# tudocomp/tudocomp

Measured on AMD Instinct MI355X. Metric: input MB/s end-to-end lcpcomp+huffman, higher is better.
Workload: dtype u32

## Files before the change

include/tdc_gpu.h:

```cpp
#ifndef TDC_GPU_H
#define TDC_GPU_H

#include <stddef.h>
#include <stdint.h>

#ifdef __cplusplus
extern "C" {
#endif

typedef enum {
    TDC_GPU_OK = 0,
    TDC_GPU_ERR_HIP = -1,
    TDC_GPU_ERR_ARG = -2,
    TDC_GPU_ERR_NO_SENTINEL = -3,
    TDC_GPU_ERR_TOO_LARGE = -4,
    TDC_GPU_ERR_OOM = -5,
    TDC_GPU_ERR_UNSUPPORTED = -6,
    TDC_GPU_ERR_INTERNAL = -7
} tdc_gpu_status;

enum { TDC_GPU_CODER_HUFF = 0, TDC_GPU_CODER_GAMMA = 1, TDC_GPU_CODER_ARITH = 2, TDC_GPU_CODER_ASCII = 3, TDC_GPU_CODER_SLE = 4,
       TDC_GPU_CODER_BIT = 5 , TDC_GPU_CODER_DELTA = 6  };
#define TDC_GPU_CODER_SLE_K(K) (TDC_GPU_CODER_SLE | ((K) << 8))
enum { TDC_GPU_COMP_ARRAYS = 0, TDC_GPU_COMP_PLCPPEAKS = 1, TDC_GPU_COMP_MAXLCP = 2, TDC_GPU_COMP_HEAP = 3 };
// ... 105 lines not shown
                                     size_t* out_len, uint64_t* factors, uint32_t* rounds);
int tdc_gpu_lzss_lcp_factorize(tdc_gpu_ctx* ctx, const uint8_t* text, size_t n, uint32_t threshold,
                               uint32_t** pos, uint32_t** src, uint32_t** len, size_t* z);

int tdc_gpu_sort_pairs_u64(tdc_gpu_ctx* ctx, uint64_t* keys, uint32_t* vals, size_t n, int algo);
int tdc_gpu_suffix_array(tdc_gpu_ctx* ctx, const uint8_t* text, size_t n, uint32_t* sa, uint32_t* isa);
int tdc_gpu_textds(tdc_gpu_ctx* ctx, const uint8_t* text, size_t n, uint32_t* sa, uint32_t* isa, uint32_t* phi,
                   uint32_t* plcp, uint32_t* lcp, uint32_t* maxlcp);
int tdc_gpu_lcpcomp_factorize(tdc_gpu_ctx* ctx, const uint8_t* text, size_t n, uint32_t threshold, int flatten,
                              uint32_t** pos, uint32_t** src, uint32_t** len, size_t* z, tdc_gpu_stats* stats);
int tdc_gpu_flatten(tdc_gpu_ctx* ctx, size_t n, const uint32_t* pos, uint32_t* src, const uint32_t* len, size_t z,
                    uint64_t* num_flattened, uint64_t* max_depth_lb);
int tdc_gpu_prim_scan(tdc_gpu_ctx* ctx, int op, void* data, size_t n, int in_place, void* total);
int tdc_gpu_prim_sort_pairs(tdc_gpu_ctx* ctx, int kind, void* keys, uint32_t* vals, size_t n, int begin_bit, int end_bit);
int tdc_gpu_prim_bucketed_scatter(tdc_gpu_ctx* ctx, const uint32_t* idx, const uint32_t* val, size_t m, uint32_t* dst, size_t n_dst,
                                  uint32_t fill, int permutation, int second_tmp, int offset);
int tdc_gpu_prim_msd_partition(tdc_gpu_ctx* ctx, uint32_t* idx, uint32_t* val, size_t m, int bits, int db);
int tdc_gpu_prim_select(tdc_gpu_ctx* ctx, const uint8_t* cls, uint8_t want, size_t m, const uint32_t* srcA, const uint64_t* srcB,
                        uint32_t fillA, uint64_t fillB, uint32_t* outA, uint64_t* outB, uint32_t* count);
int tdc_gpu_prim_select_counts(tdc_gpu_ctx* ctx, const uint8_t* cls, uint8_t want, size_t m, const uint32_t* srcA, const uint32_t* tile_counts,
                               uint32_t fillA, uint32_t* outA, uint32_t* count);
int tdc_gpu_prim_mark_orbit(tdc_gpu_ctx* ctx, const uint32_t* next, size_t n, uint8_t* mark);
int tdc_gpu_prim_tile_entries(tdc_gpu_ctx* ctx, const uint16_t* exit0, size_t ntiles, uint32_t states, uint16_t* entry0);
int tdc_gpu_prim_arena_fill(tdc_gpu_ctx* ctx, int byte, uint64_t* base, uint64_t* size);

int tdc_gpu_lcpcomp_decompress(tdc_gpu_ctx* ctx, const uint8_t* stream, size_t len, uint8_t** out, size_t* out_len,
                               uint64_t* factors, uint32_t* rounds);
int tdc_gpu_lcpcomp_decompress_coder(tdc_gpu_ctx* ctx, const uint8_t* stream, size_t len, int coder, uint8_t** out, size_t* out_len,
                                     uint64_t* factors, uint32_t* rounds);
int tdc_gpu_lcpcomp_decompress_into(tdc_gpu_ctx* ctx, const uint8_t* stream, size_t len, int coder, uint8_t* out, size_t out_cap,
                                    size_t* out_len, uint64_t* factors, uint32_t* rounds);
int tdc_gpu_ctx_last_decode_on_device(const tdc_gpu_ctx* ctx);

int tdc_gpu_lz78_decompress(tdc_gpu_ctx* ctx, const uint8_t* stream, size_t len, int coder, uint8_t** out, size_t* out_len,
                            uint64_t* phrases, uint32_t* rounds);
int tdc_gpu_lz78_decompress_into(tdc_gpu_ctx* ctx, const uint8_t* stream, size_t len, int coder, uint8_t* out, size_t out_cap,
                                 size_t* out_len, uint64_t* phrases, uint32_t* rounds);

int tdc_gpu_lzw_compress(tdc_gpu_ctx* ctx, const uint8_t* in, size_t n, int coder, uint8_t** out, size_t* out_len,
                         tdc_gpu_stats* stats);
int tdc_gpu_lzw_decompress(tdc_gpu_ctx* ctx, const uint8_t* stream, size_t len, int coder, uint8_t** out, size_t* out_len,
                           uint64_t* codes, uint32_t* rounds);
int tdc_gpu_lzw_decompress_into(tdc_gpu_ctx* ctx, const uint8_t* stream, size_t len, int coder, uint8_t* out, size_t out_cap,
                                size_t* out_len, uint64_t* codes, uint32_t* rounds);

int tdc_gpu_lzss_sw_compress(tdc_gpu_ctx* ctx, const uint8_t* in, size_t n, uint32_t window, uint32_t threshold, int coder,
// ... 113 lines not shown
```

tudocomp_amd/__init__.py:

```python
import ctypes

import numpy as np

from . import _native
from ._native import Stats, Stage, LIB_PATH, SYMBOLS

CODER_HUFF = 0
CODER_GAMMA = 1
CODER_ARITH = 2
CODER_ASCII = 3
CODER_SLE = 4
CODER_BIT = 5
CODER_DELTA = 6
COMP_ARRAYS = 0
COMP_PLCPPEAKS = 1
COMP_MAXLCP = 2
COMP_HEAP = 3
STAGE_BWT = 0
STAGE_RLE = 1
STAGE_MTF = 2
STAGE_HUFF = 3
STAGE_SLE = 4


# ... 791 lines not shown
            raise ValueError("one count per tile of 2048 classes")
        a = None if src_a is None else np.ascontiguousarray(src_a, dtype=np.uint32)
        if a is not None and len(a) != m:
            raise ValueError("cls and src_a differ in length")
        oa = np.empty(m, dtype=np.uint32)
        cnt = ctypes.c_uint32(0)
        self._check(self._L.tdc_gpu_prim_select_counts(self._h, _ptr(c), int(want), m, None if a is None else _ptr(a), _ptr(t),
                                                       int(fill_a), _ptr(oa), ctypes.byref(cnt)))
        return oa, cnt.value

    def prim_mark_orbit(self, nxt):
        a = np.ascontiguousarray(nxt, dtype=np.uint32)
        mark = np.empty(len(a), dtype=np.uint8)
        self._check(self._L.tdc_gpu_prim_mark_orbit(self._h, _ptr(a), len(a), _ptr(mark)))
        return mark

    def prim_tile_entries(self, exits):
        a = np.ascontiguousarray(exits, dtype=np.uint16)
        ntiles, states = a.shape
        entry = np.empty(ntiles, dtype=np.uint16)
        self._check(self._L.tdc_gpu_prim_tile_entries(self._h, _ptr(a), ntiles, states, _ptr(entry)))
        return entry

    def prim_arena_fill(self, byte=None):
        base, size = ctypes.c_uint64(), ctypes.c_uint64()
        self._check(self._L.tdc_gpu_prim_arena_fill(self._h, -1 if byte is None else int(byte), ctypes.byref(base), ctypes.byref(size)))
        return base.value, size.value

    def suffix_array(self, text):
        a = _u8(text)
        sa = np.empty(len(a), dtype=np.uint32)
        isa = np.empty(len(a), dtype=np.uint32)
        self._check(self._L.tdc_gpu_suffix_array(self._h, _ptr(a), len(a), _ptr(sa), _ptr(isa)))
        return sa, isa

    def textds(self, text):
        a = _u8(text)
        n = len(a)
        arrs = {k: np.empty(n, dtype=np.uint32) for k in ("sa", "isa", "phi", "plcp", "lcp")}
        m = ctypes.c_uint32()
        self._check(self._L.tdc_gpu_textds(self._h, _ptr(a), n, _ptr(arrs["sa"]), _ptr(arrs["isa"]), _ptr(arrs["phi"]),
                                           _ptr(arrs["plcp"]), _ptr(arrs["lcp"]), ctypes.byref(m)))
        arrs["maxlcp"] = m.value
        return arrs

    def lcpcomp_decompress(self, stream, coder=CODER_HUFF):
# ... 464 lines not shown
```

tudocomp_amd/_native.py:

```python
import ctypes
import os

_HERE = os.path.dirname(os.path.abspath(__file__))
LIB_PATH = os.environ.get("TDC_GPU_LIB") or os.path.join(_HERE, "lib", "libtdc_gpu.so")

SYMBOLS = [
    "tdc_gpu_ctx_create", "tdc_gpu_ctx_destroy", "tdc_gpu_ctx_reserve", "tdc_gpu_strerror", "tdc_gpu_last_error",
    "tdc_gpu_ctx_set_profiling", "tdc_gpu_ctx_reset_profile", "tdc_gpu_ctx_kernel_profile",
    "tdc_gpu_free", "tdc_gpu_lcpcomp_compress", "tdc_gpu_lcpcomp_compress_raw", "tdc_gpu_lcpcomp_compress_dev",
    "tdc_gpu_lcpcomp_bound", "tdc_gpu_lcpcomp_bound_coder", "tdc_gpu_lcpcomp_compress_into", "tdc_gpu_host_alloc", "tdc_gpu_host_free",
    "tdc_gpu_lz78_compress", "tdc_gpu_lzss_lcp_compress", "tdc_gpu_lzss_lcp_factorize",
    "tdc_gpu_sort_pairs_u64", "tdc_gpu_suffix_array", "tdc_gpu_textds", "tdc_gpu_lcpcomp_factorize", "tdc_gpu_flatten", "tdc_gpu_encode_huff",
    "tdc_gpu_prim_scan", "tdc_gpu_prim_sort_pairs", "tdc_gpu_prim_bucketed_scatter", "tdc_gpu_prim_msd_partition", "tdc_gpu_prim_select", "tdc_gpu_prim_select_counts",
    "tdc_gpu_prim_mark_orbit", "tdc_gpu_prim_tile_entries", "tdc_gpu_prim_arena_fill",
    "tdc_gpu_lcpcomp_decompress",
    "tdc_gpu_lcpcomp_compress_comp",
    "tdc_gpu_encode_arith",
    "tdc_gpu_encode_ascii",
    "tdc_gpu_encode_sle",
    "tdc_gpu_lcpcomp_decompress_coder", "tdc_gpu_ctx_last_decode_on_device", "tdc_gpu_lcpcomp_decompress_into",
    "tdc_gpu_ctx_set_option", "tdc_gpu_option_count", "tdc_gpu_option_name", "tdc_escape", "tdc_unescape", "tdc_lz78_factors", "tdc_huffman_table", "tdc_huffman_selfcheck", "tdc_gpu_blocks_count", "tdc_gpu_blocks_compress", "tdc_gpu_blocks_decompress", "tdc_gpu_device_count", "tdc_gen_english", "tdc_gen_dna",
    "tdc_gpu_arena_bytes", "tdc_gpu_device_memory",
    "tdc_gpu_lcpcomp_compress_keep", "tdc_gpu_stream_fetch", "tdc_gpu_stream_fetch_dev", "tdc_gpu_host_register", "tdc_gpu_host_unregister",
    "tdc_gpu_lz78_decompress", "tdc_gpu_lz78_decompress_into",
    "tdc_gpu_bwt_compress", "tdc_gpu_bwt_compress_into", "tdc_gpu_bwt_decompress", "tdc_gpu_bwt_decompress_into", "tdc_gpu_bwt_inverse_stage",
    "tdc_gpu_pipeline_bound", "tdc_gpu_pipeline_compress", "tdc_gpu_pipeline_compress_into", "tdc_gpu_pipeline_decompress",
    "tdc_gpu_pipeline_decompress_into", "tdc_gpu_pipeline_decompress_stats", "tdc_rle_decode", "tdc_mtf_decode", "tdc_huff_decode_literals", "tdc_sle_decode",
    "tdc_gpu_lzw_compress", "tdc_gpu_lzw_decompress", "tdc_gpu_lzw_decompress_into", "tdc_lzw_factors", "tdc_lzw_decode",
    "tdc_gpu_lzss_lcp_compress_into", "tdc_gpu_lzss_lcp_bound", "tdc_gpu_lzss_lcp_decompress", "tdc_gpu_lzss_lcp_decompress_into", "tdc_lzss_decode",
    "tdc_gpu_lzss_sw_compress", "tdc_gpu_lzss_sw_compress_into", "tdc_gpu_lzss_sw_bound", "tdc_gpu_lzss_sw_factorize", "tdc_lzss_sw_factors",
    "tdc_lzss_sw_decode", "tdc_gpu_lzss_sw_decompress", "tdc_gpu_lzss_sw_decompress_into",
    "tdc_gpu_lzss_sw_compress_batch", "tdc_gpu_lzss_sw_batch_bound", "tdc_gpu_lzss_sw_decompress_batch",
    "tdc_gpu_lzw_compress_batch", "tdc_gpu_lzw_batch_bound", "tdc_gpu_lz78_compress_batch", "tdc_gpu_lz78_batch_bound", "tdc_gpu_lz_parse_batch",
    "tdc_gpu_lzw_decompress_batch", "tdc_gpu_lz78_decompress_batch",
    "tdc_gpu_repair_compress", "tdc_gpu_repair_compress_into", "tdc_gpu_repair_bound", "tdc_gpu_repair_grammar", "tdc_gpu_repair_decompress",
    "tdc_gpu_repair_decompress_into", "tdc_gpu_repair_decompress_stats", "tdc_repair_grammar", "tdc_repair_decode",
]
# ... 81 lines not shown
    L.tdc_gpu_stream_fetch.argtypes = [vp, vp, sz, psz]
    L.tdc_gpu_stream_fetch_dev.argtypes = [vp, vp, sz, psz]
    L.tdc_gpu_ctx_last_decode_on_device.argtypes = [vp]
    L.tdc_gpu_lcpcomp_decompress_into.argtypes = [vp, vp, sz, i32, vp, sz, psz, ctypes.POINTER(ctypes.c_uint64), ctypes.POINTER(ctypes.c_uint32)]
    L.tdc_gpu_host_register.argtypes = [vp, sz]
    L.tdc_gpu_host_unregister.argtypes = [vp]
    L.tdc_gpu_blocks_count.argtypes = [sz, sz]
    L.tdc_gpu_blocks_count.restype = sz
    L.tdc_gpu_blocks_compress.argtypes = [ctypes.POINTER(i32), i32, vp, sz, sz, u32, i32, i32, pvp, psz, ctypes.POINTER(Stats)]
    L.tdc_gpu_blocks_decompress.argtypes = [vp, vp, sz, i32, pvp, psz]
    L.tdc_gpu_host_alloc.argtypes = [sz]
    L.tdc_gpu_host_alloc.restype = vp
    L.tdc_gpu_host_free.argtypes = [vp]
    L.tdc_gpu_host_free.restype = None
    L.tdc_gpu_sort_pairs_u64.argtypes = [vp, vp, vp, sz, i32]
    L.tdc_gpu_prim_scan.argtypes = [vp, i32, vp, sz, i32, vp]
    L.tdc_gpu_prim_sort_pairs.argtypes = [vp, i32, vp, vp, sz, i32, i32]
    L.tdc_gpu_prim_bucketed_scatter.argtypes = [vp, vp, vp, sz, vp, sz, u32, i32, i32, i32]
    L.tdc_gpu_prim_msd_partition.argtypes = [vp, vp, vp, sz, i32, i32]
    L.tdc_gpu_prim_select.argtypes = [vp, vp, ctypes.c_uint8, sz, vp, vp, u32, ctypes.c_uint64, vp, vp, ctypes.POINTER(u32)]
    L.tdc_gpu_prim_select_counts.argtypes = [vp, vp, ctypes.c_uint8, sz, vp, vp, u32, vp, ctypes.POINTER(u32)]
    L.tdc_gpu_prim_mark_orbit.argtypes = [vp, vp, sz, vp]
    L.tdc_gpu_prim_tile_entries.argtypes = [vp, vp, sz, u32, vp]
    L.tdc_gpu_prim_arena_fill.argtypes = [vp, i32, ctypes.POINTER(ctypes.c_uint64), ctypes.POINTER(ctypes.c_uint64)]
    L.tdc_gpu_suffix_array.argtypes = [vp, vp, sz, vp, vp]
    L.tdc_gpu_textds.argtypes = [vp, vp, sz, vp, vp, vp, vp, vp, ctypes.POINTER(u32)]
    L.tdc_gpu_lcpcomp_factorize.argtypes = [vp, vp, sz, u32, i32, pvp, pvp, pvp, psz, ctypes.POINTER(Stats)]
    L.tdc_gpu_flatten.argtypes = [vp, sz, vp, vp, vp, sz, ctypes.POINTER(ctypes.c_uint64), ctypes.POINTER(ctypes.c_uint64)]
    L.tdc_gpu_encode_huff.argtypes = [vp, vp, sz, vp, vp, vp, sz, pvp, psz]
    L.tdc_gpu_lcpcomp_decompress.argtypes = [vp, vp, sz, pvp, psz, ctypes.POINTER(ctypes.c_uint64), ctypes.POINTER(ctypes.c_uint32)]
    L.tdc_gpu_lz78_decompress.argtypes = [vp, vp, sz, i32, pvp, psz, ctypes.POINTER(ctypes.c_uint64), ctypes.POINTER(ctypes.c_uint32)]
    L.tdc_gpu_lz78_decompress_into.argtypes = [vp, vp, sz, i32, vp, sz, psz, ctypes.POINTER(ctypes.c_uint64), ctypes.POINTER(ctypes.c_uint32)]
    L.tdc_gpu_bwt_compress.argtypes = [vp, vp, sz, pvp, psz, ctypes.POINTER(Stats)]
    L.tdc_gpu_bwt_compress_into.argtypes = [vp, vp, sz, vp, sz, psz, ctypes.POINTER(Stats)]
    L.tdc_gpu_bwt_decompress.argtypes = [vp, vp, sz, pvp, psz, ctypes.POINTER(ctypes.c_uint32)]
    L.tdc_gpu_bwt_decompress_into.argtypes = [vp, vp, sz, vp, sz, psz, ctypes.POINTER(ctypes.c_uint32)]
    L.tdc_gpu_bwt_inverse_stage.argtypes = [vp, vp, sz, u32, u32, vp, vp, ctypes.POINTER(ctypes.c_uint64), ctypes.POINTER(ctypes.c_uint32)]
    pst = ctypes.POINTER(Stage)
    L.tdc_gpu_pipeline_bound.argtypes = [pst, i32, sz]
    L.tdc_gpu_pipeline_bound.restype = sz
    L.tdc_gpu_pipeline_compress.argtypes = [vp, pst, i32, vp, sz, pvp, psz, ctypes.POINTER(Stats)]
    L.tdc_gpu_pipeline_compress_into.argtypes = [vp, pst, i32, vp, sz, vp, sz, psz, ctypes.POINTER(Stats)]
    L.tdc_gpu_pipeline_decompress.argtypes = [vp, pst, i32, vp, sz, pvp, psz]
    L.tdc_gpu_pipeline_decompress_into.argtypes = [vp, pst, i32, vp, sz, vp, sz, psz]
    L.tdc_gpu_pipeline_decompress_stats.argtypes = [vp, pst, i32, vp, sz, vp, sz, psz, ctypes.POINTER(Stats)]
    L.tdc_rle_decode.argtypes = [vp, sz, ctypes.c_uint64, vp, sz, psz]
# ... 57 lines not shown
```

tudocomp_amd/csrc/api_ctx.hip:

```cpp
#include "api.hpp"
#include "huffman_host.hpp"

#include <strings.h>
#include <ctype.h>

using namespace tdc;

namespace tdc {

int lcpcomp_enc_coder(int coder) {
    const int base = coder & 0xFF, k = coder >> 8;
    if (base == TDC_GPU_CODER_SLE) {
        if (k < 0 || k > 7) throw ArgError{TDC_GPU_ERR_ARG, "sle: kmer must be in 1..7"};
        return 3 | ((k ? k : 3) << 8);
    }
    if (k == 0 && base == TDC_GPU_CODER_HUFF) return 0;
    if (k == 0 && base == TDC_GPU_CODER_ARITH) return 1;
    if (k == 0 && base == TDC_GPU_CODER_ASCII) return 2;
    throw ArgError{TDC_GPU_ERR_UNSUPPORTED, "lcpcomp: coder must be huff, arithmetic, ascii or sle"};
}

void reserve_arena(Ctx& c, size_t bytes) {
    if (c.arena.size < bytes) {
        size_t fr = 0, tot = 0;
// ... 90 lines not shown
    { "wsort_run_streams",[](Ctx& c, long v) { c.wsort_run_streams = v != 0; } },
    { "wsort_predig_skip",[](Ctx& c, long v) { c.wsort_predig_skip = clampi(v, 0, 24); } },
    { "wsort_fuse",       [](Ctx& c, long v) { c.wsort_fuse = v ? 1 : 0; } },
    { "wsort_order",      [](Ctx& c, long v) { c.wsort_order = v ? 1 : 0; } },
    { "wsort_two",        [](Ctx& c, long v) { c.wsort_two = (v >= 0 && v <= 2) ? (int)v : 0; } },
    { "wsort_leaf",       [](Ctx& c, long v) { c.wsort_leaf = v == 1024 ? 1024 : 2048; } },
    { "wsort_pack",       [](Ctx& c, long v) { c.wsort_pack = (v == 1024 || v == 4096) ? (int)v : 2048; } },
    { "wsort_cmax",       [](Ctx& c, long v) { c.wsort_cmax = clampi(v, 8, 64); } },
    { "wsort_log",        [](Ctx& c, long v) { c.wsort_log = v != 0; } },
    { "upload_chunks",    [](Ctx& c, long v) { c.upload_chunks = clampi(v, 4, 24); } },
    { "upload_tail_n",    [](Ctx& c, long v) { c.upload_tail_n = clampi(v, 0, 12); } },
    { "upload_tail_pct",  [](Ctx& c, long v) { c.upload_tail_pct = clampi(v, 30, 100); } },
    { "arena_log",        [](Ctx& c, long v) { c.arena_log = v != 0; } },
};
constexpr size_t NOPTIONS = sizeof(OPTIONS) / sizeof(OPTIONS[0]);
const OptionDef FOLD_OPTIONS[] = {
    { "fused_cand",       [](Ctx& c, long v) { c.fused_cand = v != 0; } },
    { "sel_tile_counts",  [](Ctx& c, long v) { c.sel_tile_counts = v != 0; } },
    { "flatten_chunks",   [](Ctx& c, long v) { c.flatten_chunks = clampi(v, 0, (long)FLATTEN_MAX_CHUNKS); } },
    { "repair_recount",   [](Ctx& c, long v) { c.repair_recount = v != 0; } },
    { "repair_table_bits",[](Ctx& c, long v) { c.repair_table_bits = v == 0 ? 0 : clampi(v, 8, 30); } },
    { "repair_log",       [](Ctx& c, long v) { c.repair_log = v != 0; } },
    { "repair_dec_rounds",[](Ctx& c, long v) { c.repair_dec_rounds = clampi(v, 1, 1 << 24); } },
    { "lz_batch_hash_bits",[](Ctx& c, long v) { c.lz_batch_hash_bits = clampi(v, 0, 24); } },
};
constexpr size_t NFOLD = sizeof(FOLD_OPTIONS) / sizeof(FOLD_OPTIONS[0]);
const OptionDef* find_option(const char* name) {
    if (!name) return nullptr;
    if (!strncasecmp(name, "TDC_GPU_", 8)) name += 8;
    for (size_t i = 0; i < NOPTIONS; ++i) if (!strcasecmp(name, OPTIONS[i].name)) return &OPTIONS[i];
    for (size_t i = 0; i < NFOLD; ++i) if (!strcasecmp(name, FOLD_OPTIONS[i].name)) return &FOLD_OPTIONS[i];
    return nullptr;
}
void apply_env_options(tdc_gpu_ctx* ctx) {
    const char* on = getenv("TDC_GPU_DEBUG_KNOBS");
    if (!on || atoi(on) == 0) return;
    for (size_t i = 0; i < NOPTIONS + NFOLD; ++i) {
        const OptionDef& o = i < NOPTIONS ? OPTIONS[i] : FOLD_OPTIONS[i - NOPTIONS];
        char var[64] = "TDC_GPU_";
        size_t k = 8;
        for (const char* q = o.name; *q && k + 1 < sizeof(var); ++q) var[k++] = (char)toupper((unsigned char)*q);
        var[k] = 0;
        if (const char* m = getenv(var)) o.set(ctx->c, atol(m));
    }
}
}
// ... 197 lines not shown
```

tudocomp_amd/csrc/api_prims.hip:

```cpp
#include "api.hpp"
#include "tile_chain.hpp"

#include <algorithm>
#include <vector>

using namespace tdc;

namespace {
[[noreturn]] void bad(const char* msg) { throw ArgError{TDC_GPU_ERR_ARG, msg}; }

void check_count(size_t n) {
    if (n >= 0xFFFFFFFFull) throw ArgError{TDC_GPU_ERR_TOO_LARGE, "at most 2^32 - 2 elements"};
}

template <typename T>
T* upload(Ctx& c, const T* src, size_t n, size_t offset = 0) {
    T* d = c.arena.get<T>(n + offset + 4) + offset;
    if (n) HIP_TRY(hipMemcpyAsync(d, src, n * sizeof(T), hipMemcpyHostToDevice, c.stream));
    return d;
}
template <typename T>
void download(Ctx& c, T* dst, const T* d_src, size_t n) {
    if (n) HIP_TRY(hipMemcpyAsync(dst, d_src, n * sizeof(T), hipMemcpyDeviceToHost, c.stream));
}
// ... 186 lines not shown
        u32* s1 = c.arena.get<u32>(n + 4); u32* s2 = c.arena.get<u32>(n + 4);
        mark_orbit_u32(c, d_next, n, d_mark, s1, s2);
        download(c, mark, d_mark, n);
        HIP_TRY(hipStreamSynchronize(c.stream));
    });
}

int tdc_gpu_prim_tile_entries(tdc_gpu_ctx* ctx, const uint16_t* exit0, size_t ntiles, uint32_t states, uint16_t* entry0) {
    return guarded(ctx, [&] {
        if (ntiles && (!exit0 || !entry0)) bad("exit0/entry0 is NULL");
        if (states == 0 || states >= DX_NONE) bad("1 <= states < 0xFFFF required");
        if (ntiles > ((size_t)1 << 27)) throw ArgError{TDC_GPU_ERR_TOO_LARGE, "at most 2^27 tiles"};
        for (size_t i = 0; i < ntiles * states; ++i) if (exit0[i] >= states && exit0[i] != DX_NONE) bad("every exit must be < states or 0xFFFF");
        if (ntiles == 0) return;
        Ctx& c = ctx->c;
        reserve_arena(c, 2 * ntiles * states + dx_entries_scratch((u32)ntiles, states) + ((size_t)64 << 20));
        const u16* d_exit = upload(c, exit0, ntiles * states);
        const u16* d_entry = dx_entries(c, d_exit, (u32)ntiles, states, c.arena.alloc(dx_entries_scratch((u32)ntiles, states)));
        download(c, entry0, d_entry, ntiles);
        HIP_TRY(hipStreamSynchronize(c.stream));
    });
}

int tdc_gpu_prim_arena_fill(tdc_gpu_ctx* ctx, int byte, uint64_t* base, uint64_t* size) {
    return guarded(ctx, [&] {
        if (!base || !size) bad("base/size is NULL");
        if (byte > 255) bad("byte must be 0 .. 255, or negative to fill nothing");
        Ctx& c = ctx->c;
        *base = (uint64_t)(uintptr_t)c.arena.base;
        *size = c.arena.base ? (uint64_t)c.arena.size : 0;
        if (byte < 0 || *size == 0) return;
        HIP_TRY(hipMemsetAsync(c.arena.base, byte, c.arena.size, c.stream));
        HIP_TRY(hipStreamSynchronize(c.stream));
    });
}

}
```

tudocomp_amd/csrc/common.hpp:

```cpp
#pragma once

#include <hip/hip_runtime.h>
#include <stdint.h>
#include <stddef.h>
#include <stdio.h>
#include <string.h>

namespace tdc {

typedef uint8_t  u8;
typedef uint32_t u32;
typedef uint16_t u16;
typedef uint64_t u64;

constexpr u32 NONE32 = 0xFFFFFFFFu;
constexpr int WAVE = 64;

enum {
    TDC_OK = 0,
    TDC_ERR_HIP = -1,
    TDC_ERR_ARG = -2,
    TDC_ERR_NO_SENTINEL = -3,
    TDC_ERR_TOO_LARGE = -4,
    TDC_ERR_OOM = -5,
// ... 94 lines not shown
            pinned_tab_size = bytes;
        }
        return pinned_tab;
    }
    static constexpr u32 ZC_SEG_OFF = 1040, ZC_WORDS = 1040 + 16384;
    static constexpr u32 ZC_BLOCKS = 3;
    u32* zc_host = nullptr;
    u32* zc_dev = nullptr;
    u32 zc_seq = 0;
    int fast_read = 1;
    u32* d_err = nullptr;
    int sa_local_sort = 1;
    int radix_waves = 4;
    int plcp_samples = 1;
    bool huff_ok = true;
    int flen_bytes = 1;
    int eager_levels = 1;
    int level_purge = 1;
    int enc_rec = 1;
    int owner_rem = 8;
    int enc_early = 1;
    int fused_cand = 1;
    int sel_tile_counts = 1;
    int fs_pair = 1;
    int small_big = 1;
    int small_pipeline = 1;
    int sa_pairs = 1;
    int sa_stars = 1;
    int sa_refine = 1;
    int sa_fused_init = 1;
    int radix_lds = 1;
    int xcd_remap = 1;
    int window_src = 1;
    int window_lcut = 56;
    int window_halo = 320;
    size_t dec_seg = 0;
    bool phi_lazy = true;
    int dec_lean = 1;
    int dec_parse = 1;
    int window_force_fail = 0;
    int window_large_lists = 0;
    int ssort = 1;
    int ssort_levels = 0;
    int wsort = 1;
    size_t wsort_min = (size_t)1 << 20;
    int wsort_syms = 0;
// ... 351 lines not shown
```

tudocomp_amd/csrc/fused.hip:

```cpp
#include "stages.hpp"
#include "prim.hpp"

#include <type_traits>

namespace tdc {

constexpr int FS_TILE = 4096;
constexpr int FS_ITEMS = 16;
constexpr u32 FS_WMAX = 8192;

struct FSLevel {
    const u32* idx_in; const void* rp_in; const u32* prev_in; const u8* lcp_in;
    u32* idx_out; void* rp_out; u8* lcp_out;
    u32* counts; const u32* blk_seg; const u32* blk_start; const u32* seg_start;
    u32 nseg, R, per_xcd; int shift;
    int lsh;
};
__device__ __forceinline__ bool fs_row(const FSLevel& P, u32 row, size_t& base, u32& cnt) {
    const u32 blk = row / P.R;
    if (blk >= P.blk_start[P.nseg]) return false;
    const u32 s = P.blk_seg[blk];
    const u64 t = (u64)(blk - P.blk_start[s]) * P.R + row % P.R;
    const u32 s0 = P.seg_start[s], s1 = P.seg_start[s + 1];
    const u64 off = t * FS_TILE;
// ... 16 lines not shown
    for (u32 i = threadIdx.x; i < D; i += 256) hist[i] = 0;
    if (cnt == 0) { for (u32 i = threadIdx.x; i < D; i += 256) P.counts[(size_t)row * D + i] = 0; return; }
    __syncthreads();
    const u32 lb = wave_id() * (64 * FS_ITEMS) + lane_id();
    const u32* ip = P.idx_in + base + lb;
    u32 kk[FS_ITEMS];
#pragma unroll
    for (int j = 0; j < FS_ITEMS; ++j) kk[j] = (lb + (u32)j * 64 < cnt) ? ip[j * 64] : 0u;
#pragma unroll
    for (int j = 0; j < FS_ITEMS; ++j) {
        const bool valid = lb + (u32)j * 64 < cnt;
        const u32 d = (kk[j] >> P.shift) & (D - 1);
        const u32 d0 = __builtin_amdgcn_readfirstlane(d);
        if (__all(valid && d == d0)) { if (lane_id() == 0) atomicAdd(&hist[d0], 64u); }
        else if (valid) atomicAdd(&hist[d], 1u);
    }
    __syncthreads();
    for (u32 i = threadIdx.x; i < D; i += 256) P.counts[(size_t)row * D + i] = hist[i];
}

#ifndef TDC_FS_WPE
#define TDC_FS_WPE 4
#endif
template <int DB, bool FIRST, int PAIR, bool WP>
__global__ __launch_bounds__(256 * PAIR) __attribute__((amdgpu_waves_per_eu(TDC_FS_WPE, TDC_FS_WPE))) void fs_scatter_kernel(FSLevel P, u32 rows) {
    constexpr int NT = 256 * PAIR;
    constexpr u32 TILE = (u32)FS_TILE * PAIR;
    constexpr u32 D = 1u << DB;
    __shared__ u32 tcnt[D];
    __shared__ u32 gbase[D];
    __shared__ __align__(16) u64 stage[TILE];
    __shared__ u32 scan_sm[NT / 64 + 1];
    const int lane = lane_id();
    const u32 row = xcd_tile(blockIdx.x, P.per_xcd) * PAIR;
    if (row >= rows) return;
    size_t base; u32 cnt;
    if (!fs_row(P, row, base, cnt) || cnt == 0) return;
    if (PAIR == 2 && row + 1 < rows) {
        size_t base2; u32 cnt2;
        if (fs_row(P, row + 1, base2, cnt2) && cnt2) cnt += cnt2;
    }
    for (u32 i = threadIdx.x; i < D; i += NT) tcnt[i] = 0;
    __syncthreads();
    const u32 lb = wave_id() * (64 * FS_ITEMS) + lane;
    const u32* ip = P.idx_in + base + lb;
    u32 k[FS_ITEMS], pos[FS_ITEMS];
#pragma unroll
    for (int j = 0; j < FS_ITEMS; ++j) k[j] = (lb + (u32)j * 64 < cnt) ? ip[j * 64] : 0u;
// ... 30 lines not shown
        } else if (valid) rank = atomicAdd(&tcnt[d], 1u);
        pos[j] = rank;
    }
    __syncthreads();
    {
        const u32 t = threadIdx.x;
        constexpr u32 DPT = (D + NT - 1) / NT;
        u32 tot[DPT], sum = 0;
#pragma unroll
        for (u32 q = 0; q < DPT; ++q) { const u32 d = t * DPT + q; tot[q] = d < D ? tcnt[d] : 0u; sum += tot[q]; }
        u32 total;
        u32 start = block_exclusive_sum<u32, NT / 64>(sum, scan_sm, total);
#pragma unroll
        for (u32 q = 0; q < DPT; ++q) {
            const u32 d = t * DPT + q;
            if (d < D) {
                tcnt[d] = start;
                gbase[d] = P.counts[(size_t)row * D + d] - start;
            }
            start += tot[q];
        }
    }
    __syncthreads();
    u32 dst[FS_ITEMS];
    u32* stage32 = (u32*)stage;
    unsigned short* stage_d = (unsigned short*)(stage + TILE / 2);
#pragma unroll
    for (int j = 0; j < FS_ITEMS; ++j) {
        if (lb + (u32)j * 64 < cnt) {
            const u32 d = (k[j] >> P.shift) & (D - 1);
            pos[j] += tcnt[d];
            stage32[pos[j]] = FIRST ? ((k[j] & ((1u << P.lsh) - 1u)) | (lc[j] << P.lsh)) : k[j];
            stage_d[pos[j]] = (unsigned short)d;
        }
    }
    __syncthreads();
#pragma unroll
    for (int r = 0; r < FS_ITEMS; ++r) {
        const u32 sp = (u32)r * NT + threadIdx.x;
        dst[r] = 0xFFFFFFFFu;
        if (sp < cnt) {
            dst[r] = gbase[stage_d[sp]] + sp;
            P.idx_out[dst[r]] = stage32[sp];
        }
    }
    __syncthreads();
    RT* stage2 = (RT*)stage;
#pragma unroll
    for (int j = 0; j < FS_ITEMS; ++j) if (lb + (u32)j * 64 < cnt) stage2[pos[j]] = rp[j];
    __syncthreads();
#pragma unroll
    for (int r = 0; r < FS_ITEMS; ++r) if (dst[r] != 0xFFFFFFFFu) ((RT*)P.rp_out)[dst[r]] = stage2[(u32)r * NT + threadIdx.x];
}

constexpr int FS_IMG_T = 1024;
struct FSCand { u32 threshold, lcut; u8* cls; u8* res8; u8* flen8; u32* flen; u32* tilecnt; u32* acc; };
template <bool WP, bool CF>
__global__ __launch_bounds__(FS_IMG_T) void fs_image_kernel(const u32* __restrict__ idx, const void* __restrict__ rp_v, int lsh, size_t m, u32 W,
                                                             u32* __restrict__ isa, u32* __restrict__ phi, u32* __restrict__ plcp, u32* __restrict__ d_max,
                                                             FSCand cf) {
    __shared__ __align__(16) u32 img[FS_WMAX];
    __shared__ u32 smx[FS_IMG_T / 64];
    __shared__ u32 scf[CF ? FS_IMG_T / 64 : 1];
    __shared__ u32 shist[CF ? 64 : 1];
    if (CF && threadIdx.x < 64) shist[threadIdx.x] = 0;
    constexpr int R = FS_WMAX / FS_IMG_T;
    const size_t base = (size_t)blockIdx.x * W;
    const size_t end = (base + W < m) ? base + W : m;
    using RT = typename std::conditional<WP, u64, u32>::type;
    const RT* rp = (const RT*)rp_v;
    u32 ix[R];
    RT rr[R];
    u32 mx = 0;
#pragma unroll
    for (int r = 0; r < R; ++r) {
        const size_t j = base + (size_t)r * FS_IMG_T + threadIdx.x;
        const bool have = j < end;
        ix[r] = have ? idx[j] : 0xFFFFFFFFu;
        rr[r] = have ? rp[j] : (RT)0;
    }
#pragma unroll
    for (int r = 0; r < R; ++r) if (ix[r] != 0xFFFFFFFFu) img[ix[r] & (W - 1)] = (u32)rr[r];
    __syncthreads();
#pragma unroll
    for (int r = 0; r < R; ++r) { const size_t q = base + (size_t)r * FS_IMG_T + threadIdx.x; if (q < end) isa[q] = img[q - base]; }
    __syncthreads();
    if constexpr (WP) {
#pragma unroll
        for (int r = 0; r < R; ++r) if (ix[r] != 0xFFFFFFFFu) img[ix[r] & (W - 1)] = (u32)(rr[r] >> 32);
        __syncthreads();
#pragma unroll
        for (int r = 0; r < R; ++r) { const size_t q = base + (size_t)r * FS_IMG_T + threadIdx.x; if (q < end) phi[q] = img[q - base]; }
        __syncthreads();
    }
#pragma unroll
    for (int r = 0; r < R; ++r) if (ix[r] != 0xFFFFFFFFu) { const u32 l = (ix[r] >> lsh) & 0xFFu; img[ix[r] & (W - 1)] = l; mx = max(mx, l); }
    __syncthreads();
#pragma unroll
    for (int r = 0; r < R; ++r) { const size_t q = base + (size_t)r * FS_IMG_T + threadIdx.x; if (q < end) plcp[q] = img[q - base]; }
    if constexpr (CF) {
        u32 ncand = 0;
#pragma unroll
// ... 75 lines not shown
        l = (i == 0) ? 0u : (u32)lcp8[i];
        plcp[p] = l;
    }
    l = wave_reduce_max(l);
    if (lane_id() == 0 && l) atomicMax(d_max, l);
}

bool fused_scatter_has_image(const Ctx& c, size_t n) { return n >= ((size_t)1 << 20) && c.bucket_scatter; }

void build_isa_phi_plcp_fused(Ctx& c, const u32* sa, const u8* lcp8, size_t n, u32* isa, u32* phi, u32* plcp, u32* d_maxlcp, CandFused* cf) {
    hipStream_t s = c.stream;
    if (cf) cf->filled = false;
    HIP_TRY(hipMemsetAsync(d_maxlcp, 0, sizeof(u32), s));
    if (!n) return;
    const int bits = (int)bits_for(n - 1);
    if (!fused_scatter_has_image(c, n)) {
        Ctx::ProfScope prof(c, K_PHI, (u64)n * 17);
        fs_direct_kernel<<<cdiv(n, 256), 256, 0, s>>>(sa, lcp8, n, isa, phi, plcp, d_maxlcp);
        LAUNCH_CHECK();
        return;
    }
    const size_t mark = c.arena.mark();
    const size_t m = n - 1;
    const int db = (bits - 16 > 13) ? 9 : 8;
    const u32 D = 1u << db;
    u32* idx[2] = { c.arena.get<u32>(m), c.arena.get<u32>(m) };
    const bool wp = phi != nullptr;
    void* rp[2] = { c.arena.alloc(m * (wp ? 8 : 4)), c.arena.alloc(m * (wp ? 8 : 4)) };
    const u32* seg_start = ss_first_segment(c, m);
    u32 nseg = 1;
    for (int l = 0; l < 2; ++l) {
        u32* nstart = c.arena.get<u32>((size_t)nseg * D + 1);
        const size_t lm = c.arena.mark();
        SegTables Tb;
        ss_level_tables(c, seg_start, nseg, m, D, Tb);
        FSLevel P;
        if (l == 0) { P.idx_in = sa + 1; P.rp_in = nullptr; P.prev_in = sa; P.lcp_in = lcp8 + 1; }
        else { P.idx_in = idx[0]; P.rp_in = rp[0]; P.prev_in = nullptr; P.lcp_in = nullptr; }
        P.idx_out = idx[l]; P.rp_out = rp[l]; P.lcp_out = nullptr;
        P.lsh = bits - db;
        P.counts = Tb.counts; P.blk_seg = Tb.blk_seg; P.blk_start = Tb.blk_start; P.seg_start = seg_start;
        P.nseg = nseg; P.R = Tb.R; P.shift = bits - db * (l + 1);
        const u32 rows = Tb.rows;
        P.per_xcd = (c.xcd_remap == 1 && rows >= 64) ? cdiv(rows, 8) : 0u;
        const u32 grid = P.per_xcd ? 8 * P.per_xcd : rows;
        {
            const int pc = c.prof_begin(K_RS_COUNT, (u64)m * 4);
            if (db == 9) fs_count_kernel<9><<<grid, 256, 0, s>>>(P, rows); else fs_count_kernel<8><<<grid, 256, 0, s>>>(P, rows);
            LAUNCH_CHECK();
            c.prof_end(pc);
        }
        ss_level_offsets(c, Tb, seg_start, nseg, D, nstart, m);
        {
            const int ps = c.prof_begin(K_RS_SCATTER_U32, (u64)m * (wp ? (l == 0 ? 5 + 12 : 24) : (l == 0 ? 5 + 8 : 16)));
            const bool pair = (Tb.R % 2) == 0 && c.fs_pair;
            FSLevel P2 = P;
            const u32 groups = pair ? (rows + 1) / 2 : rows;
            P2.per_xcd = (c.xcd_remap == 1 && groups >= 64) ? cdiv(groups, 8) : 0u;
            const u32 grid2 = P2.per_xcd ? 8 * P2.per_xcd : groups;
            auto launch = [&](auto wpc) {
                constexpr bool WPC = decltype(wpc)::value;
                if (pair) {
                    if (l == 0) { if (db == 9) fs_scatter_kernel<9, true, 2, WPC><<<grid2, 512, 0, s>>>(P2, rows); else fs_scatter_kernel<8, true, 2, WPC><<<grid2, 512, 0, s>>>(P2, rows); }
                    else { if (db == 9) fs_scatter_kernel<9, false, 2, WPC><<<grid2, 512, 0, s>>>(P2, rows); else fs_scatter_kernel<8, false, 2, WPC><<<grid2, 512, 0, s>>>(P2, rows); }
                } else {
                    if (l == 0) { if (db == 9) fs_scatter_kernel<9, true, 1, WPC><<<grid, 256, 0, s>>>(P, rows); else fs_scatter_kernel<8, true, 1, WPC><<<grid, 256, 0, s>>>(P, rows); }
                    else { if (db == 9) fs_scatter_kernel<9, false, 1, WPC><<<grid, 256, 0, s>>>(P, rows); else fs_scatter_kernel<8, false, 1, WPC><<<grid, 256, 0, s>>>(P, rows); }
                }
            };
            if (wp) launch(std::true_type{}); else launch(std::false_type{});
            LAUNCH_CHECK();
            c.prof_end(ps);
        }
        c.arena.release(lm);
        seg_start = nstart;
        nseg *= D;
    }
    {
        const u32 W = 1u << (bits - 2 * db);
        if (W > FS_WMAX) throw HipError{hipErrorUnknown, "fused scatter: window larger than the LDS image", (int)__LINE__};
        if (W < 16) throw HipError{hipErrorUnknown, "fused scatter: window smaller than a thread's group of positions", (int)__LINE__};
        FSCand fc{};
        if (cf) {
            if (!cf->cls || !cf->acc || !cf->lvlhist || (!cf->flen8 && !cf->flen) || (cf->lcut && !cf->res8))
                throw HipError{hipErrorUnknown, "fused scatter: candidate arrays missing", (int)__LINE__};
            fc.threshold = cf->threshold; fc.lcut = cf->lcut;
            fc.cls = cf->cls; fc.res8 = cf->lcut ? cf->res8 : nullptr; fc.flen8 = cf->flen8; fc.flen = cf->flen; fc.tilecnt = cf->tilecnt; fc.acc = cf->acc;
            HIP_TRY(hipMemsetAsync(cf->acc, 0, (size_t)CF_COPIES * CF_ACC * sizeof(u32), s));
            if (cf->tilecnt) HIP_TRY(hipMemsetAsync(cf->tilecnt, 0, (size_t)cdiv(n, SEL_TILE_CLASSES) * sizeof(u32), s));
        }
        Ctx::ProfScope prof(c, K_FS_IMAGE, (u64)m * (wp ? 24 : 16) + (cf ? (u64)m * ((cf->lcut ? 2 : 1) + (cf->flen8 ? 1 : 4)) : 0));
        if (cf) {
            if (wp) fs_image_kernel<true, true><<<cdiv(m, W), FS_IMG_T, 0, s>>>(idx[1], rp[1], bits - db, m, W, isa, phi, plcp, d_maxlcp, fc);
            else fs_image_kernel<false, true><<<cdiv(m, W), FS_IMG_T, 0, s>>>(idx[1], rp[1], bits - db, m, W, isa, phi, plcp, d_maxlcp, fc);
        } else {
            if (wp) fs_image_kernel<true, false><<<cdiv(m, W), FS_IMG_T, 0, s>>>(idx[1], rp[1], bits - db, m, W, isa, phi, plcp, d_maxlcp, fc);
            else fs_image_kernel<false, false><<<cdiv(m, W), FS_IMG_T, 0, s>>>(idx[1], rp[1], bits - db, m, W, isa, phi, plcp, d_maxlcp, fc);
        }
        LAUNCH_CHECK();
        fs_first_kernel<<<1, 1, 0, s>>>(sa, n, isa, phi, plcp, fc);
        LAUNCH_CHECK();
        if (cf) {
            fs_cand_fold_kernel<<<1, 128, 0, s>>>(cf->acc, cf->lvlhist);
            LAUNCH_CHECK();
            cf->filled = true;
        }
    }
    c.arena.release(mark);
}

}
```

Baseline: 8949.

## Pack key and payload into 8-byte records in second fused-scatter level

When Phi is not built, the second radix-scatter level now writes each key and its payload as one packed 64-bit record instead of two separate 32-bit arrays. The image kernel reads these records back with a single load per element. The aim is fewer scattered write streams and better coalescing in the final scatter and image build. It also adds a tunable digit-bit option and a test entry point for ISA/PLCP, and it relies on the arena layout holding 8-byte records in the reused buffer.

```diff
diff --git a/include/tdc_gpu.h b/include/tdc_gpu.h
--- a/include/tdc_gpu.h
+++ b/include/tdc_gpu.h
@@ -151,6 +151,7 @@
                                uint32_t fillA, uint32_t* outA, uint32_t* count);
 int tdc_gpu_prim_mark_orbit(tdc_gpu_ctx* ctx, const uint32_t* next, size_t n, uint8_t* mark);
 int tdc_gpu_prim_tile_entries(tdc_gpu_ctx* ctx, const uint16_t* exit0, size_t ntiles, uint32_t states, uint16_t* entry0);
+int tdc_gpu_prim_isa_plcp(tdc_gpu_ctx* ctx, const uint32_t* sa, const uint8_t* lcp8, size_t n, uint32_t* isa, uint32_t* plcp);
 int tdc_gpu_prim_arena_fill(tdc_gpu_ctx* ctx, int byte, uint64_t* base, uint64_t* size);
 
 int tdc_gpu_lcpcomp_decompress(tdc_gpu_ctx* ctx, const uint8_t* stream, size_t len, uint8_t** out, size_t* out_len,
diff --git a/tudocomp_amd/__init__.py b/tudocomp_amd/__init__.py
--- a/tudocomp_amd/__init__.py
+++ b/tudocomp_amd/__init__.py
@@ -837,6 +837,16 @@
         self._check(self._L.tdc_gpu_prim_tile_entries(self._h, _ptr(a), ntiles, states, _ptr(entry)))
         return entry
 
+    def prim_isa_plcp(self, sa, lcp8):
+        a = np.ascontiguousarray(sa, dtype=np.uint32)
+        l = np.ascontiguousarray(lcp8, dtype=np.uint8)
+        if len(a) != len(l):
+            raise ValueError("sa and lcp8 differ in length")
+        isa = np.empty(len(a), dtype=np.uint32)
+        plcp = np.empty(len(a), dtype=np.uint32)
+        self._check(self._L.tdc_gpu_prim_isa_plcp(self._h, _ptr(a), _ptr(l), len(a), _ptr(isa), _ptr(plcp)))
+        return isa, plcp
+
     def prim_arena_fill(self, byte=None):
         base, size = ctypes.c_uint64(), ctypes.c_uint64()
         self._check(self._L.tdc_gpu_prim_arena_fill(self._h, -1 if byte is None else int(byte), ctypes.byref(base), ctypes.byref(size)))
diff --git a/tudocomp_amd/_native.py b/tudocomp_amd/_native.py
--- a/tudocomp_amd/_native.py
+++ b/tudocomp_amd/_native.py
@@ -12,7 +12,7 @@
     "tdc_gpu_lz78_compress", "tdc_gpu_lzss_lcp_compress", "tdc_gpu_lzss_lcp_factorize",
     "tdc_gpu_sort_pairs_u64", "tdc_gpu_suffix_array", "tdc_gpu_textds", "tdc_gpu_lcpcomp_factorize", "tdc_gpu_flatten", "tdc_gpu_encode_huff",
     "tdc_gpu_prim_scan", "tdc_gpu_prim_sort_pairs", "tdc_gpu_prim_bucketed_scatter", "tdc_gpu_prim_msd_partition", "tdc_gpu_prim_select", "tdc_gpu_prim_select_counts",
-    "tdc_gpu_prim_mark_orbit", "tdc_gpu_prim_tile_entries", "tdc_gpu_prim_arena_fill",
+    "tdc_gpu_prim_mark_orbit", "tdc_gpu_prim_tile_entries", "tdc_gpu_prim_isa_plcp", "tdc_gpu_prim_arena_fill",
     "tdc_gpu_lcpcomp_decompress",
     "tdc_gpu_lcpcomp_compress_comp",
     "tdc_gpu_encode_arith",
@@ -140,6 +140,7 @@
     L.tdc_gpu_prim_select_counts.argtypes = [vp, vp, ctypes.c_uint8, sz, vp, vp, u32, vp, ctypes.POINTER(u32)]
     L.tdc_gpu_prim_mark_orbit.argtypes = [vp, vp, sz, vp]
     L.tdc_gpu_prim_tile_entries.argtypes = [vp, vp, sz, u32, vp]
+    L.tdc_gpu_prim_isa_plcp.argtypes = [vp, vp, vp, sz, vp, vp]
     L.tdc_gpu_prim_arena_fill.argtypes = [vp, i32, ctypes.POINTER(ctypes.c_uint64), ctypes.POINTER(ctypes.c_uint64)]
     L.tdc_gpu_suffix_array.argtypes = [vp, vp, sz, vp, vp]
     L.tdc_gpu_textds.argtypes = [vp, vp, sz, vp, vp, vp, vp, vp, ctypes.POINTER(u32)]
diff --git a/tudocomp_amd/csrc/api_ctx.hip b/tudocomp_amd/csrc/api_ctx.hip
--- a/tudocomp_amd/csrc/api_ctx.hip
+++ b/tudocomp_amd/csrc/api_ctx.hip
@@ -136,6 +136,8 @@
     { "repair_table_bits",[](Ctx& c, long v) { c.repair_table_bits = v == 0 ? 0 : clampi(v, 8, 30); } },
     { "repair_log",       [](Ctx& c, long v) { c.repair_log = v != 0; } },
     { "repair_dec_rounds",[](Ctx& c, long v) { c.repair_dec_rounds = clampi(v, 1, 1 << 24); } },
+    { "fs_rec64",         [](Ctx& c, long v) { c.fs_rec64 = v != 0; } },
+    { "fs_digit_bits",    [](Ctx& c, long v) { c.fs_digit_bits = (v == 8 || v == 9) ? (int)v : 0; } },
     { "lz_batch_hash_bits",[](Ctx& c, long v) { c.lz_batch_hash_bits = clampi(v, 0, 24); } },
 };
 constexpr size_t NFOLD = sizeof(FOLD_OPTIONS) / sizeof(FOLD_OPTIONS[0]);
diff --git a/tudocomp_amd/csrc/api_prims.hip b/tudocomp_amd/csrc/api_prims.hip
--- a/tudocomp_amd/csrc/api_prims.hip
+++ b/tudocomp_amd/csrc/api_prims.hip
@@ -232,6 +232,27 @@
     });
 }
 
+int tdc_gpu_prim_isa_plcp(tdc_gpu_ctx* ctx, const uint32_t* sa, const uint8_t* lcp8, size_t n, uint32_t* isa, uint32_t* plcp) {
+    return guarded(ctx, [&] {
+        if (n == 0 || !sa || !lcp8 || !isa || !plcp) bad("n is 0 or sa/lcp8/isa/plcp is NULL");
+        if (n >= ((size_t)1 << 31)) throw ArgError{TDC_GPU_ERR_TOO_LARGE, "at most 2^31 - 1 positions"};
+        if (sa[0] != n - 1) bad("sa[0] must be n - 1");
+        check_distinct_indices(sa, n, n);
+        Ctx& c = ctx->c;
+        reserve_arena(c, 64 * n + ((size_t)256 << 20));
+        const u32* d_sa = upload(c, sa, n);
+        const u8* d_lcp = upload(c, lcp8, n);
+        (void)c.arena.alloc(64);
+        u32* d_isa = c.arena.get<u32>(n + 4);
+        u32* d_plcp = c.arena.get<u32>(n + 4);
+        u32* d_max = c.arena.get<u32>(1);
+        build_isa_phi_plcp_fused(c, d_sa, d_lcp, n, d_isa, nullptr, d_plcp, d_max, nullptr);
+        download(c, isa, d_isa, n);
+        download(c, plcp, d_plcp, n);
+        HIP_TRY(hipStreamSynchronize(c.stream));
+    });
+}
+
 int tdc_gpu_prim_arena_fill(tdc_gpu_ctx* ctx, int byte, uint64_t* base, uint64_t* size) {
     return guarded(ctx, [&] {
         if (!base || !size) bad("base/size is NULL");
diff --git a/tudocomp_amd/csrc/common.hpp b/tudocomp_amd/csrc/common.hpp
--- a/tudocomp_amd/csrc/common.hpp
+++ b/tudocomp_amd/csrc/common.hpp
@@ -140,6 +140,8 @@
     int enc_early = 1;
     int fused_cand = 1;
     int sel_tile_counts = 1;
+    int fs_rec64 = 1;
+    int fs_digit_bits = 0;
     int fs_pair = 1;
     int small_big = 1;
     int small_pipeline = 1;
diff --git a/tudocomp_amd/csrc/fused.hip b/tudocomp_amd/csrc/fused.hip
--- a/tudocomp_amd/csrc/fused.hip
+++ b/tudocomp_amd/csrc/fused.hip
@@ -62,8 +62,9 @@
 #ifndef TDC_FS_WPE
 #define TDC_FS_WPE 4
 #endif
-template <int DB, bool FIRST, int PAIR, bool WP>
+template <int DB, bool FIRST, int PAIR, bool WP, bool REC = false>
 __global__ __launch_bounds__(256 * PAIR) __attribute__((amdgpu_waves_per_eu(TDC_FS_WPE, TDC_FS_WPE))) void fs_scatter_kernel(FSLevel P, u32 rows) {
+    static_assert(!REC || (!FIRST && !WP), "8-byte records: second level without Phi only");
     constexpr int NT = 256 * PAIR;
     constexpr u32 TILE = (u32)FS_TILE * PAIR;
     constexpr u32 D = 1u << DB;
@@ -140,6 +141,26 @@
         }
     }
     __syncthreads();
+    if constexpr (REC) {
+#pragma unroll
+        for (int j = 0; j < FS_ITEMS; ++j) {
+            if (lb + (u32)j * 64 < cnt) {
+                const u32 d = (k[j] >> P.shift) & (D - 1);
+                stage[pos[j] + tcnt[d]] = (u64)k[j] | ((u64)rp[j] << 32);
+            }
+        }
+        __syncthreads();
+        u64* rec_out = (u64*)P.rp_out;
+#pragma unroll
+        for (int r = 0; r < FS_ITEMS; ++r) {
+            const u32 sp = (u32)r * NT + threadIdx.x;
+            if (sp < cnt) {
+                const u64 v = stage[sp];
+                rec_out[gbase[((u32)v >> P.shift) & (D - 1)] + sp] = v;
+            }
+        }
+        return;
+    }
     u32 dst[FS_ITEMS];
     u32* stage32 = (u32*)stage;
     unsigned short* stage_d = (unsigned short*)(stage + TILE / 2);
@@ -173,7 +194,7 @@
 
 constexpr int FS_IMG_T = 1024;
 struct FSCand { u32 threshold, lcut; u8* cls; u8* res8; u8* flen8; u32* flen; u32* tilecnt; u32* acc; };
-template <bool WP, bool CF>
+template <bool WP, bool CF, bool REC = false>
 __global__ __launch_bounds__(FS_IMG_T) void fs_image_kernel(const u32* __restrict__ idx, const void* __restrict__ rp_v, int lsh, size_t m, u32 W,
                                                              u32* __restrict__ isa, u32* __restrict__ phi, u32* __restrict__ plcp, u32* __restrict__ d_max,
                                                              FSCand cf) {
@@ -181,6 +202,7 @@
     __shared__ u32 smx[FS_IMG_T / 64];
     __shared__ u32 scf[CF ? FS_IMG_T / 64 : 1];
     __shared__ u32 shist[CF ? 64 : 1];
+    static_assert(!REC || !WP, "8-byte records: without Phi only");
     if (CF && threadIdx.x < 64) shist[threadIdx.x] = 0;
     constexpr int R = FS_WMAX / FS_IMG_T;
     const size_t base = (size_t)blockIdx.x * W;
@@ -194,8 +216,14 @@
     for (int r = 0; r < R; ++r) {
         const size_t j = base + (size_t)r * FS_IMG_T + threadIdx.x;
         const bool have = j < end;
-        ix[r] = have ? idx[j] : 0xFFFFFFFFu;
-        rr[r] = have ? rp[j] : (RT)0;
+        if constexpr (REC) {
+            const u64 v = have ? ((const u64*)rp_v)[j] : 0xFFFFFFFFull;
+            ix[r] = (u32)v;
+            rr[r] = (RT)(v >> 32);
+        } else {
+            ix[r] = have ? idx[j] : 0xFFFFFFFFu;
+            rr[r] = have ? rp[j] : (RT)0;
+        }
     }
 #pragma unroll
     for (int r = 0; r < R; ++r) if (ix[r] != 0xFFFFFFFFu) img[ix[r] & (W - 1)] = (u32)rr[r];
@@ -317,11 +345,22 @@
     }
     const size_t mark = c.arena.mark();
     const size_t m = n - 1;
-    const int db = (bits - 16 > 13) ? 9 : 8;
+    int db = (bits - 16 > 13) ? 9 : 8;
+    if (c.fs_digit_bits && bits - 2 * c.fs_digit_bits >= 4 && bits - 2 * c.fs_digit_bits <= 13) db = c.fs_digit_bits;
     const u32 D = 1u << db;
-    u32* idx[2] = { c.arena.get<u32>(m), c.arena.get<u32>(m) };
     const bool wp = phi != nullptr;
-    void* rp[2] = { c.arena.alloc(m * (wp ? 8 : 4)), c.arena.alloc(m * (wp ? 8 : 4)) };
+    const bool rec = !wp && c.fs_rec64;
+    u32* idx[2]; void* rp[2];
+    idx[0] = c.arena.get<u32>(m);
+    if (rec) {
+        rp[1] = c.arena.alloc(align_up(m * 4, 256) + m * 4);
+        idx[1] = nullptr;
+        rp[0] = c.arena.alloc(m * 4);
+    } else {
+        idx[1] = c.arena.get<u32>(m);
+        rp[0] = c.arena.alloc(m * (wp ? 8 : 4));
+        rp[1] = c.arena.alloc(m * (wp ? 8 : 4));
+    }
     const u32* seg_start = ss_first_segment(c, m);
     u32 nseg = 1;
     for (int l = 0; l < 2; ++l) {
@@ -355,6 +394,11 @@
             const u32 grid2 = P2.per_xcd ? 8 * P2.per_xcd : groups;
             auto launch = [&](auto wpc) {
                 constexpr bool WPC = decltype(wpc)::value;
+                if constexpr (!WPC) if (l == 1 && rec) {
+                    if (pair) { if (db == 9) fs_scatter_kernel<9, false, 2, false, true><<<grid2, 512, 0, s>>>(P2, rows); else fs_scatter_kernel<8, false, 2, false, true><<<grid2, 512, 0, s>>>(P2, rows); }
+                    else { if (db == 9) fs_scatter_kernel<9, false, 1, false, true><<<grid, 256, 0, s>>>(P, rows); else fs_scatter_kernel<8, false, 1, false, true><<<grid, 256, 0, s>>>(P, rows); }
+                    return;
+                }
                 if (pair) {
                     if (l == 0) { if (db == 9) fs_scatter_kernel<9, true, 2, WPC><<<grid2, 512, 0, s>>>(P2, rows); else fs_scatter_kernel<8, true, 2, WPC><<<grid2, 512, 0, s>>>(P2, rows); }
                     else { if (db == 9) fs_scatter_kernel<9, false, 2, WPC><<<grid2, 512, 0, s>>>(P2, rows); else fs_scatter_kernel<8, false, 2, WPC><<<grid2, 512, 0, s>>>(P2, rows); }
@@ -385,7 +429,10 @@
             if (cf->tilecnt) HIP_TRY(hipMemsetAsync(cf->tilecnt, 0, (size_t)cdiv(n, SEL_TILE_CLASSES) * sizeof(u32), s));
         }
         Ctx::ProfScope prof(c, K_FS_IMAGE, (u64)m * (wp ? 24 : 16) + (cf ? (u64)m * ((cf->lcut ? 2 : 1) + (cf->flen8 ? 1 : 4)) : 0));
-        if (cf) {
+        if (rec) {
+            if (cf) fs_image_kernel<false, true, true><<<cdiv(m, W), FS_IMG_T, 0, s>>>(nullptr, rp[1], bits - db, m, W, isa, phi, plcp, d_maxlcp, fc);
+            else fs_image_kernel<false, false, true><<<cdiv(m, W), FS_IMG_T, 0, s>>>(nullptr, rp[1], bits - db, m, W, isa, phi, plcp, d_maxlcp, fc);
+        } else if (cf) {
             if (wp) fs_image_kernel<true, true><<<cdiv(m, W), FS_IMG_T, 0, s>>>(idx[1], rp[1], bits - db, m, W, isa, phi, plcp, d_maxlcp, fc);
             else fs_image_kernel<false, true><<<cdiv(m, W), FS_IMG_T, 0, s>>>(idx[1], rp[1], bits - db, m, W, isa, phi, plcp, d_maxlcp, fc);
         } else {
```

Result: no change. 8920 (-0.3%).
